# lightalchemist/nonlocal-image-edit

Measured on AMD Instinct MI355X. Metric: megapixels/sec end-to-end enhance (4K img, m=200, K=50); device-resident input and output (host->host per SURVEY 8d: host_to_host.value), higher is better.
Workload: dtype f64; 1 GPU; cfg4: 4096x4096 synthetic luminance, 20x10 samples (p=200), K=50, T=10, L=4 layers; device-resident: the luminance plane is in HBM when the timed region starts and the 4 layer planes are left in HBM (no PCIe inside `value`); parallelism=single GPU, formulation=phi_free_tables, storage=fp64 tables, histograms, reductions and MFMA; fp32 output planes

## Files before the change

nonlocal-image-edit_amd/csrc/sorted.hip:

```cpp
#include "sorted_rows.h"

#include <algorithm>
#include <cmath>
#include <cstdlib>

namespace nlek {

namespace {
constexpr int kSortThreads = 256;

__device__ __forceinline__ double recip0_d(double s, double eps) {
    double r = __builtin_amdgcn_rcp(s);
    r = fma(fma(-s, r, 1.0), r, r);
    r = fma(fma(-s, r, 1.0), r, r);
    return (fabs(s) >= eps) ? r : 0.0;
}

__device__ __forceinline__ int block_sum256(int v, int* red) {
#pragma unroll
    for (int off = 32; off > 0; off >>= 1) v += __shfl_xor(v, off);
    __syncthreads();
    if ((threadIdx.x & 63) == 0) red[threadIdx.x >> 6] = v;
    __syncthreads();
    return red[0] + red[1] + red[2] + red[3];
// ... 429 lines not shown
            }
            const int ns = (NC - s0 < SL) ? NC - s0 : SL;
            const int nlev = lev_nt * 16, xlo = lev_t0 * 16;
            const float inv_nlev = 1.0f / (float)nlev;
            for (int i = tid; i < ns * nlev; i += kT) {
                const int bb = (int)(((float)i + 0.5f) * inv_nlev);
                const int xx = xlo + (i - bb * nlev);
                const int f0 = sfc[xx], f1 = sfc[xx + 1];
                double sum = 0.0;
                for (int t = f0; t < f1; ++t) sum += sP[t * PS + bb];
                hrow[(size_t)(s0 + bb) * kLevels + xx] = sum;
            }
            __syncthreads();
        }
        __builtin_amdgcn_s_setprio(0);
        if (!has_next) break;
        lrow = nrow;
        nrow = nnrow;
        dsc = dsc_n;
        dsc_n = dsc_nn;
#pragma unroll
        for (int b = 0; b < kMaxBlocks; ++b) idx[b] = idx_n[b];
    }
}

int sorted_grid(int nrows, const SortedRows& sr) {
    int ncu = 256;
    int dev = 0;
    if (hipGetDevice(&dev) == hipSuccess) (void)hipDeviceGetAttribute(&ncu, hipDeviceAttributeMultiprocessorCount, dev);
    return std::max(1, std::min(nrows, sr.wgs_per_cu * ncu));
}

bool sorted_recurrence(GridSpec gs, double hx, double* kappa) {
    const double cs = gs.colStep, umax = std::max<double>(gs.colOff, gs.W - 1 - gs.colOff), nC = gs.nSelCols;
    const double span = umax + nC * cs;
    const double m_e = span * span / (hx * hx);
    const double m_rho = (2.0 * cs * umax + (2.0 * nC + 1.0) * cs * cs) / (hx * hx);
    *kappa = std::exp(-2.0 * cs * cs / (hx * hx));
    return gs.nSelCols > 12 && m_e < 500.0 && m_rho < 500.0;
}

bool sorted_moments_ok(GridSpec gs, double hx) {
    const double cs = gs.colStep, umax = std::max<double>(gs.colOff, gs.W - 1 - gs.colOff), nC = gs.nSelCols;
    const double span = umax + nC * cs;
    return span * span / (hx * hx) < 500.0;
}

hipError_t sorted_pass(hipStream_t s, int mode, GridSpec gs, int row0, int nrows_local, const SortedRows& sr, const double* d_g,
                       double eps, double* d_ybuf, double* d_h, const double* d_cvec, const float* d_xvec) {
    const int nC = gs.nSelCols, lev_t0 = sr.lev_t0, lev_nt = sr.lev_nt;
    if (!tables_apply(gs) || gs.W > sorted_max_width() || lev_t0 < 0 || lev_nt < 1 || lev_t0 + lev_nt > kLevels / 16)
        return hipErrorInvalidValue;
    if (nrows_local <= 0) return hipSuccess;
    const size_t shm = sorted_lds_bytes(gs.W, (nC < 11 ? nC : 11) | 1);
    const int grid = sorted_grid(nrows_local, sr);
#define NLE_SP1(NCV, CFV)                                                                                                 \
    {                                                                                                                     \
        if (shm > 48 * 1024) {                                                                                            \
            hipError_t ea = hipFuncSetAttribute(reinterpret_cast<const void*>(k_sorted_pass<NCV, CFV>),                   \
                                                hipFuncAttributeMaxDynamicSharedMemorySize, (int)shm);                    \
            if (ea != hipSuccess) return ea;                                                                              \
        }                                                                                                                 \
        hipLaunchKernelGGL((k_sorted_pass<NCV, CFV>), dim3((unsigned)grid), dim3(kT), shm, s, mode, sr.scol, sr.desc,      \
                           sr.first, gs, row0, nrows_local, sr.E, d_g, eps, d_ybuf, d_h, d_cvec, d_xvec, sr.kappa, lev_t0, \
                           lev_nt);                                                                                       \
    }
#define NLE_SP(NCV)                                                                                                       \
    case NCV:                                                                                                             \
        if constexpr ((NCV) > 1) {                                                                                        \
            if (sr.mom) {                                                                                                 \
                NLE_SP1(NCV, 2)                                                                                           \
                break;                                                                                                    \
            }                                                                                                             \
        }                                                                                                                 \
        if constexpr ((NCV) > 12) {                                                                                       \
            if (sr.rec) NLE_SP1(NCV, 1) else NLE_SP1(NCV, 0)                                                              \
        } else {                                                                                                          \
            if (sr.rec) return hipErrorInvalidValue;                                                                      \
            NLE_SP1(NCV, 0)                                                                                               \
        }                                                                                                                 \
        break;
    switch (nC) {
        NLE_SP(1) NLE_SP(2) NLE_SP(3) NLE_SP(4) NLE_SP(5) NLE_SP(6) NLE_SP(7) NLE_SP(8) NLE_SP(9) NLE_SP(10) NLE_SP(11)
        NLE_SP(12) NLE_SP(13) NLE_SP(14) NLE_SP(15) NLE_SP(16) NLE_SP(17) NLE_SP(18) NLE_SP(19) NLE_SP(20)
        NLE_SP(21) NLE_SP(22) NLE_SP(23) NLE_SP(24) NLE_SP(25) NLE_SP(26) NLE_SP(27) NLE_SP(28) NLE_SP(29)
        NLE_SP(30) NLE_SP(31) NLE_SP(32) NLE_SP(33) NLE_SP(34) NLE_SP(35) NLE_SP(36)
        default: return hipErrorInvalidValue;
    }
#undef NLE_SP
#undef NLE_SP1
    return hipGetLastError();
}

constexpr int kExpLayers = 4;
template <int NC, int kExpL, bool REC>
__global__ __launch_bounds__(kT) void k_sorted_expand(const unsigned short* __restrict__ scol, const uint2* __restrict__ desc,
                                                      GridSpec gs, int nrows, const double* __restrict__ Etab,
                                                      const double* __restrict__ g, size_t gstride, int nl,
                                                      const double* __restrict__ cvec, float* __restrict__ out,
                                                      long long ostride, double kappa, int round8) {
    extern __shared__ __attribute__((aligned(16))) unsigned char smem_raw[];
    constexpr int n = kLevels * NC;
    const int W = gs.W;
    double* sE = reinterpret_cast<double*>(smem_raw);
    float* sOut = reinterpret_cast<float*>(sE + ((W + 2) & ~1));
    const int tid = threadIdx.x;
    for (int i = tid; i <= W; i += kT) sE[i] = Etab[i];
    const int cb0 = gs.colOff, cs = gs.colStep;
    const unsigned sEa = lds_addr(sE);
    const size_t pitch = sorted_row_pitch(W);
    __syncthreads();
    for (int lrow = blockIdx.x; lrow < nrows; lrow += gridDim.x) {
        const uint2 dsc = desc[(size_t)lrow * kT + tid];
        const int len = dsc_len(dsc), x = dsc_level(dsc);
        const uint2* slot = reinterpret_cast<const uint2*>(scol + (size_t)lrow * pitch + (size_t)tid * dsc_chp(dsc));
        uint2 idx[kMaxBlocks];
#pragma unroll
        for (int b = 0; b < kMaxBlocks; ++b) {
            uint2 v = make_uint2(0u, 0u);
            if (4 * b < len) v = slot[b];
            idx[b] = v;
        }
        double gv[kExpL][NC];
#pragma unroll
        for (int l = 0; l < kExpL; ++l)
#pragma unroll
            for (int b = 0; b < NC; ++b) gv[l][b] = (l < nl) ? g[(size_t)l * gstride + (size_t)lrow * n + b * kLevels + x] : 0.0;
        const double* cv_row = cvec + (size_t)lrow * W;
        int wlen = len;
#pragma unroll
        for (int off = 32; off > 0; off >>= 1) wlen = max(wlen, __shfl_xor(wlen, off));
        wlen = __builtin_amdgcn_readfirstlane(wlen);
        auto pixel = [&](const unsigned c8, const bool on) {
            const unsigned c = c8 >> 3;
            const double cv = cv_row[c];
            double e[NC];
            column_factors<NC, REC>(sEa, c8, cb0, cs, kappa, [&](const int b, const double ev) { e[b] = ev; });
#pragma unroll
            for (int l = 0; l < kExpL; ++l) {
                double s0 = 0.0, s1 = 0.0;
#pragma unroll
                for (int b = 0; b < NC; ++b) {
                    if (b & 1) s1 += e[b] * gv[l][b];
                    else s0 += e[b] * gv[l][b];
                }
                if (on && l < nl) {
                    double v = cv * (s0 + s1);
                    if (round8) v = rint(fmin(255.0, fmax(0.0, v)));
                    sOut[l * W + c] = (float)v;
                }
            }
        };
#pragma unroll
        for (int b = 0; b < kMaxBlocks; ++b) {
            if (4 * b >= wlen) break;
            pixel(idx[b].x & 0xffffu, 4 * b < len);
            NLE_PIXEL_FENCE();
            if (4 * b + 1 < wlen) {
                pixel(idx[b].x >> 16, 4 * b + 1 < len);
                NLE_PIXEL_FENCE();
            }
            if (4 * b + 2 < wlen) {
                pixel(idx[b].y & 0xffffu, 4 * b + 2 < len);
                NLE_PIXEL_FENCE();
            }
            if (4 * b + 3 < wlen) {
                pixel(idx[b].y >> 16, 4 * b + 3 < len);
                NLE_PIXEL_FENCE();
            }
        }
        __syncthreads();
        for (int l = 0; l < nl; ++l) {
            float* orow = out + (size_t)l * ostride + (size_t)lrow * W;
            for (int c = tid; c < W; c += kT) orow[c] = sOut[l * W + c];
        }
        __syncthreads();
    }
}

int sorted_expand_layers(GridSpec gs) { return (gs.nSelCols <= 12 && gs.W <= 4096) ? kExpLayers : 2; }

hipError_t sorted_expand(hipStream_t s, GridSpec gs, int nrows_local, const SortedRows& sr, const double* d_g, size_t gstride,
                         int nl, const double* d_cvec, float* d_out, long long ostride, bool round8) {
    const int nC = gs.nSelCols;
    const int lmax = sorted_expand_layers(gs);
    if (!tables_apply(gs) || gs.W > sorted_max_width() || nl < 1 || nl > lmax) return hipErrorInvalidValue;
    if (nrows_local <= 0) return hipSuccess;
    const size_t shm = (size_t)((gs.W + 2) & ~1) * sizeof(double) + (size_t)lmax * gs.W * sizeof(float);
    int ncu = 256, dev = 0;
    if (hipGetDevice(&dev) == hipSuccess) (void)hipDeviceGetAttribute(&ncu, hipDeviceAttributeMultiprocessorCount, dev);
    const int grid = std::max(1, std::min(nrows_local, ncu));
#define NLE_SX1(NCV, LV, RECV)                                                                                         \
    {                                                                                                                  \
        if (shm > 48 * 1024) {                                                                                         \
            hipError_t ea = hipFuncSetAttribute(reinterpret_cast<const void*>(k_sorted_expand<NCV, LV, RECV>),         \
                                                hipFuncAttributeMaxDynamicSharedMemorySize, (int)shm);                 \
            if (ea != hipSuccess) return ea;                                                                           \
        }                                                                                                              \
        hipLaunchKernelGGL((k_sorted_expand<NCV, LV, RECV>), dim3((unsigned)grid), dim3(kT), shm, s, sr.scol, sr.desc, \
                           gs, nrows_local, sr.E, d_g, gstride, nl, d_cvec, d_out, ostride, sr.kappa, round8 ? 1 : 0); \
    }
#define NLE_SX(NCV)                                                                                                    \
    case NCV:                                                                                                          \
        if constexpr ((NCV) <= 12) {                                                                                   \
            if (lmax == kExpLayers) NLE_SX1(NCV, kExpLayers, false) else NLE_SX1(NCV, 2, false)                        \
        } else {                                                                                                       \
            if (sr.rec) NLE_SX1(NCV, 2, true) else NLE_SX1(NCV, 2, false)                                              \
        }                                                                                                              \
        break;
    switch (nC) {
        NLE_SX(1) NLE_SX(2) NLE_SX(3) NLE_SX(4) NLE_SX(5) NLE_SX(6) NLE_SX(7) NLE_SX(8) NLE_SX(9) NLE_SX(10) NLE_SX(11)
        NLE_SX(12) NLE_SX(13) NLE_SX(14) NLE_SX(15) NLE_SX(16) NLE_SX(17) NLE_SX(18) NLE_SX(19) NLE_SX(20) NLE_SX(21)
        NLE_SX(22) NLE_SX(23) NLE_SX(24) NLE_SX(25) NLE_SX(26) NLE_SX(27) NLE_SX(28) NLE_SX(29) NLE_SX(30) NLE_SX(31)
        NLE_SX(32) NLE_SX(33) NLE_SX(34) NLE_SX(35) NLE_SX(36)
        default: return hipErrorInvalidValue;
    }
#undef NLE_SX
#undef NLE_SX1
    return hipGetLastError();
}

template <int NC, bool REC>
__global__ __launch_bounds__(kT) void k_sorted_gram(const unsigned short* __restrict__ scol, const uint2* __restrict__ desc,
                                                    const unsigned short* __restrict__ first, GridSpec gs, int nrows,
                                                    const double* __restrict__ Etab, const double* __restrict__ cvec,
                                                    double* __restrict__ Aout, double kappa) {
    extern __shared__ __attribute__((aligned(16))) unsigned char smem_raw[];
    constexpr int NP = NC * (NC + 1) / 2;
    constexpr int SL = 11, PS = SL;
// ... 305 lines not shown
```

nonlocal-image-edit_amd/csrc/sorted_planes.hip:

```cpp
#include "sorted_rows.h"

#include <algorithm>

namespace nlek {

__host__ __device__ constexpr int planes_waves_per_simd(int nc, int np) { return nc * np <= 28 ? 4 : 2; }

template <int NC, int CF, int NP>
__global__ __launch_bounds__(kT, planes_waves_per_simd(NC, NP)) void k_sorted_reduce_planes(
    const unsigned short* __restrict__ scol, const uint2* __restrict__ desc, const unsigned short* __restrict__ first, GridSpec gs,
    int row0, int nrows, const double* __restrict__ Etab, const double* __restrict__ cvec, PlaneGroup pg, double kappa,
    int lev_t0, int lev_nt) {
#pragma clang fp contract(off)
    extern __shared__ __attribute__((aligned(16))) unsigned char smem_raw[];
    constexpr int n = kLevels * NC;
    constexpr int SL = NC < 11 ? NC : 11;
    constexpr int PS = SL | 1;
    constexpr bool REC = CF == 1, MOM = CF == 2;
    static_assert(!MOM || NC > 1, "the moment form needs two columns");
    const int W = gs.W;
    const size_t pitch = sorted_row_pitch(W);
    double* sE = reinterpret_cast<double*>(smem_raw);
    double* sP = sE + ((W + 2) & ~1);
    unsigned short* sfirst = reinterpret_cast<unsigned short*>(sP + (size_t)kT * PS);
    double* sCk = reinterpret_cast<double*>(sfirst + 2 * 260);
    const int tid = threadIdx.x;
    for (int i = tid; i <= W; i += kT) sE[i] = Etab[i];
    if (MOM && tid == 0) {
        double ck = 1.0, kp = 1.0;
        for (int b = 0; b < NC; ++b) {
            sCk[b] = ck;
            ck *= kp;
            kp *= kappa;
        }
    }
    const int cb0 = gs.colOff, cs = gs.colStep;
    const unsigned sEa = lds_addr(sE);

    const int G = (int)gridDim.x;
    int lrow = blockIdx.x, nrow = lrow + G;
    uint2 dsc = desc[(size_t)lrow * kT + tid];
    uint2 dsc_n = dsc;
    if (nrow < nrows) dsc_n = desc[(size_t)nrow * kT + tid];
    if (tid < 258) sfirst[tid] = first[(size_t)lrow * 258 + tid];
    uint2 idx[kMaxBlocks];
    auto load_idx = [&](uint2 (&dst)[kMaxBlocks], const int row, const uint2 d) {
        const uint2* slot = reinterpret_cast<const uint2*>(scol + (size_t)row * pitch + (size_t)tid * dsc_chp(d));
        const int ln = dsc_len(d);
#pragma unroll
        for (int b = 0; b < kMaxBlocks; ++b) {
            uint2 v = make_uint2(0u, 0u);
            if (4 * b < ln) v = slot[b];
            dst[b] = v;
        }
    };
    load_idx(idx, lrow, dsc);
    __syncthreads();
    for (int par = 0;; par ^= 1) {
        const bool has_next = nrow < nrows;
        const int nnrow = nrow + G;
        const unsigned short* sfc = sfirst + par * 260;
        const int len = dsc_len(dsc);
        double acc[NP][NC];
#pragma unroll
        for (int m = 0; m < NP; ++m)
#pragma unroll
            for (int b = 0; b < NC; ++b) acc[m][b] = 0.0;
        const double* cv_row = cvec + (size_t)lrow * W;
        const float* xv_row[NP];
#pragma unroll
        for (int m = 0; m < NP; ++m) xv_row[m] = pg.x[m] + (size_t)(row0 + lrow) * W;
        uint2 dsc_nn = dsc_n;
        unsigned short sf_n = 0;
        uint2 idx_n[kMaxBlocks];
        if (has_next) {
            if (nnrow < nrows) dsc_nn = desc[(size_t)nnrow * kT + tid];
            sf_n = first[(size_t)nrow * 258 + (tid < 258 ? tid : 257)];
            load_idx(idx_n, nrow, dsc_n);
        }
        auto pixel_mom = [&](const unsigned c8, const int at) {
            if constexpr (!MOM) return;
            else {
                const double e0 = e_at(sEa, c8, (unsigned)cb0 << 3);
                double rho = e_at(sEa, c8, (unsigned)(cb0 + cs) << 3);
                const bool keep = at < len;
                const double cv = cv_row[c8 >> 3];
                float xs[NP];
#pragma unroll
                for (int m = 0; m < NP; ++m) xs[m] = xv_row[m][c8 >> 3];
                double r0 = __builtin_amdgcn_rcp(e0);
                r0 = fma(fma(-e0, r0, 1.0), r0, r0);
                r0 = fma(fma(-e0, r0, 1.0), r0, r0);
                rho = rho * r0;
                const double rho2 = rho * rho;
#pragma unroll
                for (int m = 0; m < NP; ++m) {
                    double y = cv * (double)xs[m];
                    y = keep ? y : 0.0;
                    double te = y * e0;
                    acc[m][0] = fma(y, e0, acc[m][0]);
                    double to = te * rho;
                    acc[m][1] = fma(te, rho, acc[m][1]);
#pragma unroll
                    for (int b = 2; b < NC; b += 2) {
                        acc[m][b] = fma(te, rho2, acc[m][b]);
                        te = te * rho2;
                        if (b + 1 < NC) {
                            acc[m][b + 1] = fma(to, rho2, acc[m][b + 1]);
                            to = to * rho2;
                        }
                    }
                }
            }
        };
        auto pixel = [&](const unsigned c8, const bool on) {
            const double cv = cv_row[c8 >> 3];
            double y[NP];
#pragma unroll
            for (int m = 0; m < NP; ++m) {
                const double v = cv * (double)xv_row[m][c8 >> 3];
                y[m] = on ? v : 0.0;
            }
            column_factors<NC, REC>(sEa, c8, cb0, cs, kappa, [&](const int b, const double ev) {
#pragma unroll
                for (int m = 0; m < NP; ++m) acc[m][b] = fma(ev, y[m], acc[m][b]);
            });
        };
        int wlen = len;
#pragma unroll
        for (int off = 32; off > 0; off >>= 1) wlen = max(wlen, __shfl_xor(wlen, off));
        wlen = __builtin_amdgcn_readfirstlane(wlen);
#pragma unroll
        for (int b = 0; b < kMaxBlocks; ++b) {
            if (4 * b >= wlen) break;
            const unsigned cs4[4] = {idx[b].x & 0xffffu, idx[b].x >> 16, idx[b].y & 0xffffu, idx[b].y >> 16};
#pragma unroll
            for (int k = 0; k < 4; ++k) {
                if (4 * b + k < wlen) {
                    if constexpr (MOM) pixel_mom(cs4[k], 4 * b + k);
                    else pixel(cs4[k], 4 * b + k < len);
                    NLE_PIXEL_FENCE();
                }
            }
        }
        if constexpr (MOM) {
#pragma unroll
            for (int m = 0; m < NP; ++m)
#pragma unroll
                for (int b = 2; b < NC; ++b) acc[m][b] = acc[m][b] * sCk[b];
        }
        __builtin_amdgcn_s_setprio(3);
        const int nlev = lev_nt * 16, xlo = lev_t0 * 16;
        const float inv_nlev = 1.0f / (float)nlev;
#pragma unroll
        for (int m = 0; m < NP; ++m) {
            double* hrow = pg.h[m] + (size_t)lrow * n;
#pragma unroll
            for (int s0 = 0; s0 < NC; s0 += SL) {
#pragma unroll
                for (int i = 0; i < SL; ++i) sP[tid * PS + i] = (s0 + i < NC) ? acc[m][s0 + i] : 0.0;
                __syncthreads();
                if (m == 0 && s0 == 0) {
                    asm volatile("" ::"v"(sf_n), "v"(dsc_nn.x), "v"(dsc_nn.y));
#pragma unroll
                    for (int b = 0; b < kMaxBlocks; ++b) asm volatile("" ::"v"(idx_n[b].x), "v"(idx_n[b].y));
                    if (has_next && tid < 258) sfirst[(par ^ 1) * 260 + tid] = sf_n;
                }
                const int ns = (NC - s0 < SL) ? NC - s0 : SL;
                for (int i = tid; i < ns * nlev; i += kT) {
                    const int bb = (int)(((float)i + 0.5f) * inv_nlev);
                    const int xx = xlo + (i - bb * nlev);
                    const int f0 = sfc[xx], f1 = sfc[xx + 1];
                    double sum = 0.0;
                    for (int t = f0; t < f1; ++t) sum += sP[t * PS + bb];
                    hrow[(size_t)(s0 + bb) * kLevels + xx] = sum;
                }
                __syncthreads();
            }
        }
        __builtin_amdgcn_s_setprio(0);
        if (!has_next) break;
        lrow = nrow;
        nrow = nnrow;
        dsc = dsc_n;
        dsc_n = dsc_nn;
#pragma unroll
        for (int b = 0; b < kMaxBlocks; ++b) idx[b] = idx_n[b];
    }
}

int sorted_planes_per_launch(GridSpec gs) { return gs.nSelCols <= 12 ? kPlanesPerLaunch : 2; }

hipError_t sorted_reduce_planes(hipStream_t s, GridSpec gs, int row0, int nrows_local, const SortedRows& sr, const double* d_cvec,
                                const PlaneGroup& pg, int np) {
    const int nC = gs.nSelCols, lev_t0 = sr.lev_t0, lev_nt = sr.lev_nt;
    if (!tables_apply(gs) || gs.W > sorted_max_width() || lev_t0 < 0 || lev_nt < 1 || lev_t0 + lev_nt > kLevels / 16 || np < 2 ||
        np > sorted_planes_per_launch(gs))
        return hipErrorInvalidValue;
    if (nrows_local <= 0) return hipSuccess;
    const size_t shm = sorted_lds_bytes(gs.W, (nC < 11 ? nC : 11) | 1);
    SortedRows one = sr;
    if (planes_waves_per_simd(nC, np) < 4) one.wgs_per_cu = 1;
    const int grid = sorted_grid(nrows_local, one);
#define NLE_RP1(NCV, CFV, NPV)                                                                                            \
    {                                                                                                                     \
        if (shm > 48 * 1024) {                                                                                            \
            hipError_t ea = hipFuncSetAttribute(reinterpret_cast<const void*>(k_sorted_reduce_planes<NCV, CFV, NPV>),     \
                                                hipFuncAttributeMaxDynamicSharedMemorySize, (int)shm);                    \
            if (ea != hipSuccess) return ea;                                                                              \
        }                                                                                                                 \
        hipLaunchKernelGGL((k_sorted_reduce_planes<NCV, CFV, NPV>), dim3((unsigned)grid), dim3(kT), shm, s, sr.scol,       \
                           sr.desc, sr.first, gs, row0, nrows_local, sr.E, d_cvec, pg, sr.kappa, lev_t0, lev_nt);         \
    }
#define NLE_RPN(NCV, CFV)                                                                                                 \
    {                                                                                                                     \
        if constexpr ((NCV) <= 12) {                                                                                      \
            if (np == 4) NLE_RP1(NCV, CFV, 4) else if (np == 3) NLE_RP1(NCV, CFV, 3) else NLE_RP1(NCV, CFV, 2)            \
        } else {                                                                                                          \
            NLE_RP1(NCV, CFV, 2)                                                                                          \
        }                                                                                                                 \
    }
#define NLE_RP(NCV)                                                                                                       \
    case NCV:                                                                                                             \
        if constexpr ((NCV) > 1) {                                                                                        \
            if (sr.mom) {                                                                                                 \
                NLE_RPN(NCV, 2)                                                                                           \
                break;                                                                                                    \
            }                                                                                                             \
        }                                                                                                                 \
        if constexpr ((NCV) > 12) {                                                                                       \
            if (sr.rec) NLE_RPN(NCV, 1) else NLE_RPN(NCV, 0)                                                              \
        } else {                                                                                                          \
            if (sr.rec) return hipErrorInvalidValue;                                                                      \
            NLE_RPN(NCV, 0)                                                                                               \
        }                                                                                                                 \
        break;
    switch (nC) {
        NLE_RP(1) NLE_RP(2) NLE_RP(3) NLE_RP(4) NLE_RP(5) NLE_RP(6) NLE_RP(7) NLE_RP(8) NLE_RP(9) NLE_RP(10) NLE_RP(11)
        NLE_RP(12) NLE_RP(13) NLE_RP(14) NLE_RP(15) NLE_RP(16) NLE_RP(17) NLE_RP(18) NLE_RP(19) NLE_RP(20)
        NLE_RP(21) NLE_RP(22) NLE_RP(23) NLE_RP(24) NLE_RP(25) NLE_RP(26) NLE_RP(27) NLE_RP(28) NLE_RP(29)
        NLE_RP(30) NLE_RP(31) NLE_RP(32) NLE_RP(33) NLE_RP(34) NLE_RP(35) NLE_RP(36)
        default: return hipErrorInvalidValue;
    }
#undef NLE_RP
#undef NLE_RPN
#undef NLE_RP1
    return hipGetLastError();
}

}
```

nonlocal-image-edit_amd/csrc/tables.hip:

```cpp
#include "kernels.h"

#include <algorithm>

namespace nlek {

typedef double f64x4 __attribute__((ext_vector_type(4)));

constexpr int kLevels = 256;

constexpr int kGroupMin = 12;
constexpr int kGroupRounds = 3;

template <int CTRL, int ROW_MASK>
__device__ __forceinline__ double dpp_f64(double v) {
    int lo = __double2loint(v), hi = __double2hiint(v);
    lo = __builtin_amdgcn_update_dpp(0, lo, CTRL, ROW_MASK, 0xf, true);
    hi = __builtin_amdgcn_update_dpp(0, hi, CTRL, ROW_MASK, 0xf, true);
    return __hiloint2double(hi, lo);
}
__device__ __forceinline__ double wave_sum63(double v) {
    v += dpp_f64<0xB1, 0xf>(v);
    v += dpp_f64<0x4E, 0xf>(v);
    v += dpp_f64<0x141, 0xf>(v);
    v += dpp_f64<0x140, 0xf>(v);
// ... 51 lines not shown
    __shared__ int s_bad[4];
    if ((threadIdx.x & 63) == 0) {
        s_tiles[threadIdx.x >> 6] = tiles;
        s_bad[threadIdx.x >> 6] = any_bad ? 1 : 0;
    }
    __syncthreads();
    if (threadIdx.x == 0) {
        if (s_bad[0] | s_bad[1] | s_bad[2] | s_bad[3]) atomicOr(flag, 1);
        atomicOr(flag + 1, (int)(s_tiles[0] | s_tiles[1] | s_tiles[2] | s_tiles[3]));
    }
}

hipError_t check_levels(hipStream_t s, const float* d_lum, long long n, int* d_flag) {
    hipError_t e = hipMemsetAsync(d_flag, 0, 2 * sizeof(int), s);
    if (e != hipSuccess) return e;
    long long g = (n + 255) / 256;
    if (g > 1024) g = 1024;
    hipLaunchKernelGGL(k_check_levels, dim3((unsigned)g), dim3(256), 0, s, d_lum, n, d_flag);
    return hipGetLastError();
}

__global__ void k_hist_tables(GridSpec gs, const Sample4* __restrict__ samples, int p, double inv_hx2,
                              double inv_hy2, int row0, int nrows_local, double* __restrict__ er,
                              double* __restrict__ ecT, double* __restrict__ Ep) {
    const long long n_er = (long long)nrows_local * gs.nSelRows, n_ec = (long long)gs.nSelCols * gs.W,
                    n_ep = (long long)kLevels * p;
    for (long long i = (long long)blockIdx.x * blockDim.x + threadIdx.x; i < n_er + n_ec + n_ep;
         i += (long long)gridDim.x * blockDim.x) {
        if (i < n_er) {
            const int r = row0 + (int)(i / gs.nSelRows), a = (int)(i % gs.nSelRows);
            const double d = (double)(r - (gs.rowOff + a * gs.rowStep));
            er[i] = exp(-(d * d) * inv_hx2);
        } else if (i < n_er + n_ec) {
            const long long j = i - n_er;
            const int b = (int)(j / gs.W), c = (int)(j % gs.W);
            const double d = (double)(c - (gs.colOff + b * gs.colStep));
            ecT[j] = exp(-(d * d) * inv_hx2);
        } else {
            const long long j = i - n_er - n_ec;
            const int x = (int)(j / p), sidx = (int)(j % p);
            const double d = (double)x - (double)samples[sidx].z;
            Ep[j] = exp(-(d * d) * inv_hy2);
        }
    }
}

hipError_t hist_tables(hipStream_t s, GridSpec gs, const Sample4* d_samples, int p, double hx, double hy, int row0,
                       int nrows_local, double* d_er, double* d_ecT, double* d_Ep) {
    hipLaunchKernelGGL(k_hist_tables, dim3(256), dim3(256), 0, s, gs, d_samples, p, 1.0 / (hx * hx), 1.0 / (hy * hy),
                       row0, nrows_local, d_er, d_ecT, d_Ep);
    return hipGetLastError();
}

__global__ __launch_bounds__(256) void k_hist_g(GridSpec gs, int p, int nrows, int tiles_per_wave, int lev_t0, int lev_nt,
                                                const double* __restrict__ er, const double* __restrict__ Ep,
                                                const double* __restrict__ w, double* __restrict__ g) {
    extern __shared__ __attribute__((aligned(16))) unsigned char smem_raw[];
    double* sEr = reinterpret_cast<double*>(smem_raw);
    const int nC = gs.nSelCols, nR = gs.nSelRows, n = kLevels * nC;
    const int tid = threadIdx.x, lane = tid & 63, wave = tid >> 6, l15 = lane & 15, kq = lane >> 4;
    const int t0 = blockIdx.y * tiles_per_wave, ntiles = (nrows + 15) >> 4;
    const int rbase = t0 * 16, rcount = min(nrows - rbase, tiles_per_wave * 16);
    for (int i = tid; i < rcount * nR; i += 256) sEr[i] = er[(size_t)rbase * nR + i];
    const int q = blockIdx.x * 4 + wave;
    const bool col_ok = q < nC * lev_nt;
    const int b = col_ok ? q / lev_nt : 0, x = (lev_t0 + (col_ok ? q % lev_nt : 0)) * 16 + l15;
    const int col = b * kLevels + x;
    double bop[8];
#pragma unroll
    for (int ks = 0; ks < 8; ++ks) {
        const int a = ks * 4 + kq;
        bop[ks] = (col_ok && a < nR) ? w[a * nC + b] * Ep[(size_t)x * p + a * nC + b] : 0.0;
    }
    __syncthreads();
    if (!col_ok) return;
    const int ksteps = (nR + 3) >> 2;
    for (int t = t0; t < min(ntiles, t0 + tiles_per_wave); ++t) {
        const int rl = (t - t0) * 16 + l15;
        double aop[8];
#pragma unroll
        for (int ks = 0; ks < 8; ++ks) {
            const int a = ks * 4 + kq;
            aop[ks] = (ks < ksteps && rl < rcount && a < nR) ? sEr[rl * nR + a] : 0.0;
        }
        f64x4 acc = f64x4{0.0, 0.0, 0.0, 0.0};
#pragma unroll
        for (int ks = 0; ks < 8; ++ks)
            if (ks < ksteps) acc = __builtin_amdgcn_mfma_f64_16x16x4f64(aop[ks], bop[ks], acc, 0, 0, 0);
        if (col_ok) {
#pragma unroll
            for (int e = 0; e < 4; ++e) {
                const int ro = t * 16 + kq + 4 * e;
                if (ro < nrows) g[(size_t)ro * n + col] = acc[e];
            }
        }
    }
}

static hipError_t launch_hist_g(hipStream_t s, GridSpec gs, int p, int nrows_local, const double* d_er, const double* d_Ep,
                                const double* d_w, double* d_g, int lev_t0 = 0, int lev_nt = kLevels / 16) {
    const int ntiles = (nrows_local + 15) / 16;
    const int gx = (gs.nSelCols * lev_nt + 3) / 4;
    const int cap = gs.nSelRows > 24 ? 8 : 16;
    const int chunks = std::max(1, std::min(ntiles, std::max((640 + gx - 1) / gx, (ntiles + cap - 1) / cap)));
    const int tpw = (ntiles + chunks - 1) / chunks;
    const size_t shm = (size_t)tpw * 16 * gs.nSelRows * sizeof(double);
    if (shm > 48 * 1024) {
        hipError_t ea = hipFuncSetAttribute(reinterpret_cast<const void*>(k_hist_g), hipFuncAttributeMaxDynamicSharedMemorySize,
                                            (int)shm);
        if (ea != hipSuccess) return ea;
    }
    hipLaunchKernelGGL(k_hist_g, dim3((unsigned)gx, (unsigned)((ntiles + tpw - 1) / tpw)), dim3(256), shm, s, gs, p,
                       nrows_local, tpw, lev_t0, lev_nt, d_er, d_Ep, d_w, d_g);
    return hipGetLastError();
}

constexpr int kPixThreads = 512;
template <int NC>
__global__ __launch_bounds__(kPixThreads) void k_hist_pix(int mode, const float* __restrict__ lum, GridSpec gs, int row0,
                                                  const double* __restrict__ ecT, const double* __restrict__ g,
                                                  double eps, double* __restrict__ ybuf, double* __restrict__ hout,
                                                  const double* __restrict__ cvec, const float* __restrict__ xvec) {
    extern __shared__ __attribute__((aligned(16))) unsigned char smem_raw[];
    constexpr int n = kLevels * NC;
    constexpr int NS = NC | 1;
    const int W = gs.W;
    double* sg = reinterpret_cast<double*>(smem_raw);
    double* sh = sg + kLevels * NS;
    const int tid = threadIdx.x, lrow = blockIdx.x, r = row0 + lrow;
    const double* grow = g + (size_t)lrow * n;
    for (int i = tid; i < n; i += kPixThreads) {
        const int bb = i / kLevels, xx = i & (kLevels - 1);
        sh[xx * NS + bb] = 0.0;
        sg[xx * NS + bb] = (mode == ROWPASS_RECIP) ? grow[i] : 0.0;
    }
    __syncthreads();
    const int dr = r - gs.rowOff;
    const bool sample_row = dr >= 0 && (dr % gs.rowStep) == 0 && (dr / gs.rowStep) < gs.nSelRows;
    for (int c0 = 0; c0 < W; c0 += kPixThreads) {
        const bool inside = c0 + tid < W;
        const int c = inside ? c0 + tid : W - 1;
        const int x = (int)lum[(size_t)r * W + c];
        bool smp = !inside;
        if (sample_row) {
            const int dc = c - gs.colOff;
            smp = smp || (dc >= 0 && (dc % gs.colStep) == 0 && (dc / gs.colStep) < NC);
        }
        double e[NC];
#pragma unroll
        for (int b = 0; b < NC; ++b) e[b] = ecT[(size_t)b * W + c];
        double y = 1.0;
        if (mode == ROWPASS_XVEC) {
            y = cvec[(size_t)lrow * W + c] * (double)xvec[(size_t)r * W + c];
        } else if (mode == ROWPASS_RECIP) {
            double gv[NC];
#pragma unroll
            for (int b = 0; b < NC; ++b) gv[b] = sg[x * NS + b];
            double s0 = 0.0, s1 = 0.0;
#pragma unroll
            for (int b = 0; b < NC; ++b) {
                if (b & 1) s1 += e[b] * gv[b];
                else s0 += e[b] * gv[b];
            }
            y = recip_or_zero_d(s0 + s1, eps);
        }
        if (smp) y = 0.0;
// ... 275 lines not shown
        }
        switch (nC) {
            NLE_HP(1) NLE_HP(2) NLE_HP(3) NLE_HP(4) NLE_HP(5) NLE_HP(6) NLE_HP(7) NLE_HP(8) NLE_HP(9) NLE_HP(10) NLE_HP(11)
            NLE_HP(12) NLE_HP(13) NLE_HP(14) NLE_HP(15) NLE_HP(16) NLE_HP(17) NLE_HP(18) NLE_HP(19) NLE_HP(20)
            NLE_HP(21) NLE_HP(22) NLE_HP(23) NLE_HP(24) NLE_HP(25) NLE_HP(26) NLE_HP(27) NLE_HP(28) NLE_HP(29)
            NLE_HP(30) NLE_HP(31) NLE_HP(32) NLE_HP(33) NLE_HP(34) NLE_HP(35) NLE_HP(36)
            default: return hipErrorInvalidValue;
        }
#undef NLE_HP
    }
    Scope sc(obs, SUB_HIST_HH);
    return launch_hist_hh_z(s, v, d_h, d_HH, d_z);
}

size_t apply_reduce_planes_workspace_elems(GridSpec gs, int nrows_local, int np) {
    return hist_tiled_workspace_elems(gs, nrows_local) + (size_t)std::max(np - 2, 0) * nrows_local * kLevels * gs.nSelCols;
}

hipError_t apply_reduce_planes(hipStream_t s, const TableView& v, const float* const* d_x, int np, double* d_ws, double* d_m,
                               LaunchObserver* obs) {
    if (!tables_apply(v.gs) || v.sorted == nullptr || np < 2 || np > sorted_planes_per_launch(v.gs)) return hipErrorInvalidValue;
    const size_t tab = (size_t)v.nrows * kLevels * v.gs.nSelCols;
    double* d_HH = d_ws + (size_t)np * tab;
    PlaneGroup pg{};
    for (int m = 0; m < np; ++m) pg.x[m] = d_x[m], pg.h[m] = d_ws + (size_t)m * tab;
    if (obs) obs->begin(SUB_HIST_PIX);
    hipError_t ep = sorted_reduce_planes(s, v.gs, v.row0, v.nrows, *v.sorted, v.cvec, pg, np);
    if (obs) obs->end();
    if (ep != hipSuccess) return ep;
    for (int m = 0; m < np; ++m) {
        if (obs) obs->begin(SUB_HIST_HH);
        hipError_t eh = launch_hist_hh_z(s, v, pg.h[m], d_HH, d_m + (size_t)m * v.ldp);
        if (obs) obs->end();
        if (eh != hipSuccess) return eh;
    }
    return hipSuccess;
}

int apply_layers_per_launch(const TableView& v) {
    if (v.sorted != nullptr) return sorted_expand_layers(v.gs);
    const size_t table = (size_t)kLevels * (v.gs.nSelCols | 1) * sizeof(double);
    return (int)std::max<size_t>(1, std::min<size_t>(kDotLayers, (size_t)(144 * 1024) / table));
}

hipError_t apply_hist_layers(hipStream_t s, const TableView& v, const double* d_wl, int ldw, int nl, double* d_ws, float* d_out,
                             long long ostride, LaunchObserver* obs, bool round8) {
    if (v.nrows <= 0) return hipSuccess;
    if (!tables_apply(v.gs) || nl < 1 || nl > apply_layers_per_launch(v)) return hipErrorInvalidValue;
    const GridSpec gs = v.gs;
    const int nC = gs.nSelCols, p = v.p, row0 = v.row0, nrows_local = v.nrows;
    const SortedRows* sorted = v.sorted;
    const size_t n = (size_t)kLevels * nC, gstride = (size_t)nrows_local * n;
    if (obs) obs->begin(SUB_HIST_G);
    for (int l = 0; l < nl; ++l) {
        hipError_t eg = launch_hist_g(s, gs, p, nrows_local, v.er, v.Ep, d_wl + (size_t)l * ldw, d_ws + (size_t)l * gstride,
                                      sorted ? sorted->lev_t0 : 0, sorted ? sorted->lev_nt : kLevels / 16);
        if (eg != hipSuccess) return eg;
    }
    if (obs) obs->end(), obs->begin(SUB_HIST_PIX);
    if (sorted != nullptr) {
        hipError_t ex = sorted_expand(s, gs, nrows_local, *sorted, d_ws, gstride, nl, v.cvec, d_out, ostride, round8);
        if (obs) obs->end();
        return ex;
    }
#define NLE_HD(NCV)                                                                                                  \
    case NCV: {                                                                                                      \
        const size_t shm_d = (size_t)nl * kLevels * ((NCV) | 1) * sizeof(double);                                    \
        if (shm_d > 48 * 1024) {                                                                                     \
            hipError_t ea = hipFuncSetAttribute(reinterpret_cast<const void*>(k_hist_dot<NCV>),                      \
                                                hipFuncAttributeMaxDynamicSharedMemorySize, (int)shm_d);             \
            if (ea != hipSuccess) return ea;                                                                         \
        }                                                                                                            \
        hipLaunchKernelGGL((k_hist_dot<NCV>), dim3((unsigned)nrows_local), dim3(kDotThreads), shm_d, s, v.lum, gs,   \
                           row0, v.ecT, d_ws, gstride, nl, v.cvec, d_out, ostride, round8 ? 1 : 0);                  \
    } break;
    switch (nC) {
        NLE_HD(1) NLE_HD(2) NLE_HD(3) NLE_HD(4) NLE_HD(5) NLE_HD(6) NLE_HD(7) NLE_HD(8) NLE_HD(9) NLE_HD(10) NLE_HD(11)
        NLE_HD(12) NLE_HD(13) NLE_HD(14) NLE_HD(15) NLE_HD(16) NLE_HD(17) NLE_HD(18) NLE_HD(19) NLE_HD(20)
        NLE_HD(21) NLE_HD(22) NLE_HD(23) NLE_HD(24) NLE_HD(25) NLE_HD(26) NLE_HD(27) NLE_HD(28) NLE_HD(29)
        NLE_HD(30) NLE_HD(31) NLE_HD(32) NLE_HD(33) NLE_HD(34) NLE_HD(35) NLE_HD(36)
        default: return hipErrorInvalidValue;
    }
#undef NLE_HD
    if (obs) obs->end();
    return hipGetLastError();
}

hipError_t apply_small(hipStream_t s, int p, int K, int ldk, int L, int ldw, const double* d_m, const double* d_D,
                       const double* d_Vrows, const double* d_xA, const double* d_resp, double* d_t, double* d_Wp,
                       double* d_YA) {
    const size_t shm = (size_t)(2 * p + K + 256) * sizeof(double);
    hipLaunchKernelGGL(k_apply_small, dim3((unsigned)L), dim3(256), shm, s, p, K, ldk, L, ldw, d_m, d_D, d_Vrows, d_xA,
                       d_resp, d_t, d_Wp, d_YA);
    return hipGetLastError();
}

hipError_t scatter_samples(hipStream_t s, int p, int L, const long long* d_loc, const double* d_YA, float* d_Y,
                           long long ystride, bool round8) {
    hipLaunchKernelGGL(k_scatter_samples, dim3((unsigned)((L * p + 255) / 256)), dim3(256), 0, s, p, L, d_loc, d_YA, d_Y,
                       ystride, round8 ? 1 : 0);
    return hipGetLastError();
}

__device__ __forceinline__ int tri_index(int i, int j, int n) {
    return i * n - (i * (i - 1)) / 2 + (j - i);
}

constexpr int kGhistRowsThreads = 512;
__global__ __launch_bounds__(kGhistRowsThreads) void k_ghist_rows(const float* __restrict__ lum, GridSpec gs, int row0,
// ... 362 lines not shown
```

Before: 3460 MP/s.

## Prefetch cvec/x gathers ahead in sorted kernels and batch hist_g across layers

The sorted expand kernel now software-pipelines the next row's descriptor, index, g-table and cvec gathers so they load while the current row's pixels are computed. The single-plane XVEC row pass is routed through the planes reducer, which gains an NP=1 path that gathers cvec and x one block ahead. k_hist_g is templated on layer count so up to 4 layers share one launch and one Ep load. These changes aim to hide gather latency and cut launches, at the cost of more registers and possible occupancy loss.

After: 3471 MP/s, median of 2. No clear change (+0.3%).

```diff
diff --git a/nonlocal-image-edit_amd/csrc/sorted.hip b/nonlocal-image-edit_amd/csrc/sorted.hip
--- a/nonlocal-image-edit_amd/csrc/sorted.hip
+++ b/nonlocal-image-edit_amd/csrc/sorted.hip
@@ -505,6 +505,12 @@
     if (!tables_apply(gs) || gs.W > sorted_max_width() || lev_t0 < 0 || lev_nt < 1 || lev_t0 + lev_nt > kLevels / 16)
         return hipErrorInvalidValue;
     if (nrows_local <= 0) return hipSuccess;
+    if (mode == ROWPASS_XVEC) {
+        if (d_cvec == nullptr || d_xvec == nullptr || d_ybuf != nullptr) return hipErrorInvalidValue;
+        PlaneGroup pg{};
+        pg.x[0] = d_xvec, pg.h[0] = d_h;
+        return sorted_reduce_planes(s, gs, row0, nrows_local, sr, d_cvec, pg, 1);
+    }
     const size_t shm = sorted_lds_bytes(gs.W, (nC < 11 ? nC : 11) | 1);
     const int grid = sorted_grid(nrows_local, sr);
 #define NLE_SP1(NCV, CFV)                                                                                                 \
@@ -554,6 +560,10 @@
                                                       long long ostride, double kappa, int round8) {
     extern __shared__ __attribute__((aligned(16))) unsigned char smem_raw[];
     constexpr int n = kLevels * NC;
+    constexpr int NB = kExpL == kExpLayers ? 4 : kMaxBlocks;
+    constexpr bool PIPE = NC <= 29 || (NC == 30 && REC);
+    constexpr bool CVALL = NC <= 12;
+    constexpr int NCR = CVALL ? 4 * NB : 4;
     const int W = gs.W;
     double* sE = reinterpret_cast<double*>(smem_raw);
     float* sOut = reinterpret_cast<float*>(sE + ((W + 2) & ~1));
@@ -562,31 +572,87 @@
     const int cb0 = gs.colOff, cs = gs.colStep;
     const unsigned sEa = lds_addr(sE);
     const size_t pitch = sorted_row_pitch(W);
-    __syncthreads();
-    for (int lrow = blockIdx.x; lrow < nrows; lrow += gridDim.x) {
-        const uint2 dsc = desc[(size_t)lrow * kT + tid];
-        const int len = dsc_len(dsc), x = dsc_level(dsc);
-        const uint2* slot = reinterpret_cast<const uint2*>(scol + (size_t)lrow * pitch + (size_t)tid * dsc_chp(dsc));
-        uint2 idx[kMaxBlocks];
-#pragma unroll
-        for (int b = 0; b < kMaxBlocks; ++b) {
+    auto load_idx = [&](uint2 (&dst)[NB], const int row, const uint2 d) {
+        const uint2* slot = reinterpret_cast<const uint2*>(scol + (size_t)row * pitch + (size_t)tid * dsc_chp(d));
+        const int ln = dsc_len(d);
+#pragma unroll
+        for (int b = 0; b < NB; ++b) {
             uint2 v = make_uint2(0u, 0u);
-            if (4 * b < len) v = slot[b];
-            idx[b] = v;
-        }
-        double gv[kExpL][NC];
-#pragma unroll
-        for (int l = 0; l < kExpL; ++l)
-#pragma unroll
-            for (int b = 0; b < NC; ++b) gv[l][b] = (l < nl) ? g[(size_t)l * gstride + (size_t)lrow * n + b * kLevels + x] : 0.0;
+            if (4 * b < ln) v = slot[b];
+            dst[b] = v;
+        }
+    };
+    auto load_gv = [&](double (&dst)[kExpL][NC], const int row, const uint2 d) {
+        const double* gx = g + (size_t)row * n + dsc_level(d);
+#pragma unroll
+        for (int l = 0; l < kExpL; ++l) {
+            const double* gl = gx + (l < nl ? (size_t)l * gstride : (size_t)0);
+#pragma unroll
+            for (int b = 0; b < NC; ++b) dst[l][b] = gl[b * kLevels];
+        }
+    };
+    auto gather4 = [&](double* dst, const double* cv_row, const uint2 ix) {
+        dst[0] = cv_row[(ix.x & 0xffffu) >> 3];
+        dst[1] = cv_row[ix.x >> 19];
+        dst[2] = cv_row[(ix.y & 0xffffu) >> 3];
+        dst[3] = cv_row[ix.y >> 19];
+    };
+    auto gather_first = [&](double (&dst)[NCR], const int row, const uint2 (&ix)[NB], const int wl) {
+        const double* cv_row = cvec + (size_t)row * W;
+#pragma unroll
+        for (int b = 0; b < (CVALL ? NB : 1); ++b) {
+            if (4 * b >= wl) break;
+            gather4(&dst[4 * b], cv_row, ix[b]);
+        }
+    };
+    auto wave_len = [&](const uint2 d) {
+        int wl = dsc_len(d);
+#pragma unroll
+        for (int off = 32; off > 0; off >>= 1) wl = max(wl, __shfl_xor(wl, off));
+        return __builtin_amdgcn_readfirstlane(wl);
+    };
+    const int G = (int)gridDim.x;
+    int lrow = blockIdx.x, nrow = lrow + G;
+    uint2 dsc = desc[(size_t)lrow * kT + tid];
+    uint2 dsc_n = dsc;
+    if constexpr (PIPE) {
+        if (nrow < nrows) dsc_n = desc[(size_t)nrow * kT + tid];
+    }
+    uint2 idx[NB];
+    load_idx(idx, lrow, dsc);
+    int wlen = wave_len(dsc);
+    double cvr[NCR];
+    if constexpr (PIPE) gather_first(cvr, lrow, idx, wlen);
+    double gv[kExpL][NC];
+    load_gv(gv, lrow, dsc);
+    __syncthreads();
+    for (;;) {
+        const bool has_next = nrow < nrows;
+        const int nnrow = nrow + G;
+        const int len = dsc_len(dsc);
+        uint2 dsc_nn = dsc_n;
+        uint2 idx_n[PIPE ? NB : 1];
+        if constexpr (PIPE) {
+#pragma unroll
+            for (int l = 0; l < kExpL; ++l)
+#pragma unroll
+                for (int b = 0; b < NC; ++b) asm volatile("" ::"v"(gv[l][b]));
+#pragma unroll
+            for (int i = 0; i < NCR; ++i) {
+                if (4 * (i / 4) < wlen) asm volatile("" ::"v"(cvr[i]));
+            }
+            if (has_next) {
+                if (nnrow < nrows) dsc_nn = desc[(size_t)nnrow * kT + tid];
+                load_idx(idx_n, nrow, dsc_n);
+            } else {
+#pragma unroll
+                for (int b = 0; b < NB; ++b) idx_n[b] = make_uint2(0u, 0u);
+            }
+        }
         const double* cv_row = cvec + (size_t)lrow * W;
-        int wlen = len;
-#pragma unroll
-        for (int off = 32; off > 0; off >>= 1) wlen = max(wlen, __shfl_xor(wlen, off));
-        wlen = __builtin_amdgcn_readfirstlane(wlen);
-        auto pixel = [&](const unsigned c8, const bool on) {
+        auto pixel = [&](const unsigned c8, const bool on, const double cv_reg) {
             const unsigned c = c8 >> 3;
-            const double cv = cv_row[c];
+            const double cv = PIPE ? cv_reg : cv_row[c];
             double e[NC];
             column_factors<NC, REC>(sEa, c8, cb0, cs, kappa, [&](const int b, const double ev) { e[b] = ev; });
 #pragma unroll
@@ -605,21 +671,44 @@
             }
         };
 #pragma unroll
-        for (int b = 0; b < kMaxBlocks; ++b) {
+        for (int b = 0; b < NB; ++b) {
             if (4 * b >= wlen) break;
-            pixel(idx[b].x & 0xffffu, 4 * b < len);
+            double cvb[4];
+            if constexpr (PIPE && !CVALL) {
+                if (b + 1 < NB && 4 * (b + 1) < wlen) gather4(cvb, cv_row, idx[b + 1]);
+            }
+            double cv4[4] = {0.0, 0.0, 0.0, 0.0};
+            if constexpr (PIPE) {
+#pragma unroll
+                for (int k = 0; k < 4; ++k) cv4[k] = cvr[(CVALL ? 4 * b : 0) + k];
+            }
+            pixel(idx[b].x & 0xffffu, 4 * b < len, cv4[0]);
             NLE_PIXEL_FENCE();
             if (4 * b + 1 < wlen) {
-                pixel(idx[b].x >> 16, 4 * b + 1 < len);
+                pixel(idx[b].x >> 16, 4 * b + 1 < len, cv4[1]);
                 NLE_PIXEL_FENCE();
             }
             if (4 * b + 2 < wlen) {
-                pixel(idx[b].y & 0xffffu, 4 * b + 2 < len);
+                pixel(idx[b].y & 0xffffu, 4 * b + 2 < len, cv4[2]);
                 NLE_PIXEL_FENCE();
             }
             if (4 * b + 3 < wlen) {
-                pixel(idx[b].y >> 16, 4 * b + 3 < len);
+                pixel(idx[b].y >> 16, 4 * b + 3 < len, cv4[3]);
                 NLE_PIXEL_FENCE();
+            }
+            if constexpr (PIPE && !CVALL) {
+                if (b + 1 < NB && 4 * (b + 1) < wlen) {
+#pragma unroll
+                    for (int k = 0; k < 4; ++k) cvr[k] = cvb[k];
+                }
+            }
+        }
+        int wlen_n = 0;
+        if constexpr (PIPE) {
+            if (has_next) {
+                wlen_n = wave_len(dsc_n);
+                gather_first(cvr, nrow, idx_n, wlen_n);
+                load_gv(gv, nrow, dsc_n);
             }
         }
         __syncthreads();
@@ -628,6 +717,21 @@
             for (int c = tid; c < W; c += kT) orow[c] = sOut[l * W + c];
         }
         __syncthreads();
+        if (!has_next) break;
+        lrow = nrow;
+        nrow = nnrow;
+        if constexpr (PIPE) {
+            dsc = dsc_n;
+            dsc_n = dsc_nn;
+            wlen = wlen_n;
+#pragma unroll
+            for (int b = 0; b < NB; ++b) idx[b] = idx_n[b];
+        } else {
+            dsc = desc[(size_t)lrow * kT + tid];
+            load_idx(idx, lrow, dsc);
+            load_gv(gv, lrow, dsc);
+            wlen = wave_len(dsc);
+        }
     }
 }
 
diff --git a/nonlocal-image-edit_amd/csrc/sorted_planes.hip b/nonlocal-image-edit_amd/csrc/sorted_planes.hip
--- a/nonlocal-image-edit_amd/csrc/sorted_planes.hip
+++ b/nonlocal-image-edit_amd/csrc/sorted_planes.hip
@@ -4,7 +4,7 @@
 
 namespace nlek {
 
-__host__ __device__ constexpr int planes_waves_per_simd(int nc, int np) { return nc * np <= 28 ? 4 : 2; }
+__host__ __device__ constexpr int planes_waves_per_simd(int nc, int np) { return np == 1 ? (nc <= 12 ? 4 : 2) : (nc * np <= 28 ? 4 : 2); }
 
 template <int NC, int CF, int NP>
 __global__ __launch_bounds__(kT, planes_waves_per_simd(NC, NP)) void k_sorted_reduce_planes(
@@ -55,6 +55,31 @@
         }
     };
     load_idx(idx, lrow, dsc);
+    constexpr bool AHEAD = NP == 1;
+    auto gather4 = [&](double (&cv)[4], float (&xs)[NP][4], const int row, const uint2 ix) {
+        const unsigned c4[4] = {(ix.x & 0xffffu) >> 3, ix.x >> 19, (ix.y & 0xffffu) >> 3, ix.y >> 19};
+        const double* cv_row = cvec + (size_t)row * W;
+#pragma unroll
+        for (int k = 0; k < 4; ++k) cv[k] = cv_row[c4[k]];
+#pragma unroll
+        for (int m = 0; m < NP; ++m) {
+            const float* xv_row = pg.x[m] + (size_t)(row0 + row) * W;
+#pragma unroll
+            for (int k = 0; k < 4; ++k) xs[m][k] = xv_row[c4[k]];
+        }
+    };
+    auto wave_len = [&](const uint2 d) {
+        int wl = dsc_len(d);
+#pragma unroll
+        for (int off = 32; off > 0; off >>= 1) wl = max(wl, __shfl_xor(wl, off));
+        return __builtin_amdgcn_readfirstlane(wl);
+    };
+    int wlen = wave_len(dsc);
+    double cvc[4] = {};
+    float xsc[NP][4] = {};
+    if constexpr (AHEAD) {
+        if (wlen > 0) gather4(cvc, xsc, lrow, idx[0]);
+    }
     __syncthreads();
     for (int par = 0;; par ^= 1) {
         const bool has_next = nrow < nrows;
@@ -70,6 +95,14 @@
         const float* xv_row[NP];
 #pragma unroll
         for (int m = 0; m < NP; ++m) xv_row[m] = pg.x[m] + (size_t)(row0 + lrow) * W;
+        if (AHEAD && wlen > 0) {
+#pragma unroll
+            for (int k = 0; k < 4; ++k) {
+                asm volatile("" ::"v"(cvc[k]));
+#pragma unroll
+                for (int m = 0; m < NP; ++m) asm volatile("" ::"v"(xsc[m][k]));
+            }
+        }
         uint2 dsc_nn = dsc_n;
         unsigned short sf_n = 0;
         uint2 idx_n[kMaxBlocks];
@@ -78,16 +111,21 @@
             sf_n = first[(size_t)nrow * 258 + (tid < 258 ? tid : 257)];
             load_idx(idx_n, nrow, dsc_n);
         }
-        auto pixel_mom = [&](const unsigned c8, const int at) {
+        auto pixel_mom = [&](const unsigned c8, const int at, const double cva, const float (&xsa)[NP]) {
             if constexpr (!MOM) return;
             else {
                 const double e0 = e_at(sEa, c8, (unsigned)cb0 << 3);
                 double rho = e_at(sEa, c8, (unsigned)(cb0 + cs) << 3);
                 const bool keep = at < len;
-                const double cv = cv_row[c8 >> 3];
+                double cv = cva;
                 float xs[NP];
 #pragma unroll
-                for (int m = 0; m < NP; ++m) xs[m] = xv_row[m][c8 >> 3];
+                for (int m = 0; m < NP; ++m) xs[m] = xsa[m];
+                if constexpr (!AHEAD) {
+                    cv = cv_row[c8 >> 3];
+#pragma unroll
+                    for (int m = 0; m < NP; ++m) xs[m] = xv_row[m][c8 >> 3];
+                }
                 double r0 = __builtin_amdgcn_rcp(e0);
                 r0 = fma(fma(-e0, r0, 1.0), r0, r0);
                 r0 = fma(fma(-e0, r0, 1.0), r0, r0);
@@ -113,12 +151,15 @@
                 }
             }
         };
-        auto pixel = [&](const unsigned c8, const bool on) {
-            const double cv = cv_row[c8 >> 3];
+        auto pixel = [&](const unsigned c8, const bool on, const double cva, const float (&xsa)[NP]) {
+            double cv = cva;
+            if constexpr (!AHEAD) cv = cv_row[c8 >> 3];
             double y[NP];
 #pragma unroll
             for (int m = 0; m < NP; ++m) {
-                const double v = cv * (double)xv_row[m][c8 >> 3];
+                float x = xsa[m];
+                if constexpr (!AHEAD) x = xv_row[m][c8 >> 3];
+                const double v = cv * (double)x;
                 y[m] = on ? v : 0.0;
             }
             column_factors<NC, REC>(sEa, c8, cb0, cs, kappa, [&](const int b, const double ev) {
@@ -126,20 +167,31 @@
                 for (int m = 0; m < NP; ++m) acc[m][b] = fma(ev, y[m], acc[m][b]);
             });
         };
-        int wlen = len;
-#pragma unroll
-        for (int off = 32; off > 0; off >>= 1) wlen = max(wlen, __shfl_xor(wlen, off));
-        wlen = __builtin_amdgcn_readfirstlane(wlen);
 #pragma unroll
         for (int b = 0; b < kMaxBlocks; ++b) {
             if (4 * b >= wlen) break;
+            const bool more = AHEAD && b + 1 < kMaxBlocks && 4 * (b + 1) < wlen;
+            double cvn[4];
+            float xsn[NP][4];
+            if (more) gather4(cvn, xsn, lrow, idx[b + 1]);
             const unsigned cs4[4] = {idx[b].x & 0xffffu, idx[b].x >> 16, idx[b].y & 0xffffu, idx[b].y >> 16};
 #pragma unroll
             for (int k = 0; k < 4; ++k) {
                 if (4 * b + k < wlen) {
-                    if constexpr (MOM) pixel_mom(cs4[k], 4 * b + k);
-                    else pixel(cs4[k], 4 * b + k < len);
+                    float xs[NP];
+#pragma unroll
+                    for (int m = 0; m < NP; ++m) xs[m] = xsc[m][k];
+                    if constexpr (MOM) pixel_mom(cs4[k], 4 * b + k, cvc[k], xs);
+                    else pixel(cs4[k], 4 * b + k < len, cvc[k], xs);
                     NLE_PIXEL_FENCE();
+                }
+            }
+            if (more) {
+#pragma unroll
+                for (int k = 0; k < 4; ++k) {
+                    cvc[k] = cvn[k];
+#pragma unroll
+                    for (int m = 0; m < NP; ++m) xsc[m][k] = xsn[m][k];
                 }
             }
         }
@@ -152,6 +204,7 @@
         __builtin_amdgcn_s_setprio(3);
         const int nlev = lev_nt * 16, xlo = lev_t0 * 16;
         const float inv_nlev = 1.0f / (float)nlev;
+        const int wlen_n = wave_len(dsc_n);
 #pragma unroll
         for (int m = 0; m < NP; ++m) {
             double* hrow = pg.h[m] + (size_t)lrow * n;
@@ -165,6 +218,7 @@
 #pragma unroll
                     for (int b = 0; b < kMaxBlocks; ++b) asm volatile("" ::"v"(idx_n[b].x), "v"(idx_n[b].y));
                     if (has_next && tid < 258) sfirst[(par ^ 1) * 260 + tid] = sf_n;
+                    if (AHEAD && has_next && wlen_n > 0) gather4(cvc, xsc, nrow, idx_n[0]);
                 }
                 const int ns = (NC - s0 < SL) ? NC - s0 : SL;
                 for (int i = tid; i < ns * nlev; i += kT) {
@@ -184,6 +238,7 @@
         nrow = nnrow;
         dsc = dsc_n;
         dsc_n = dsc_nn;
+        wlen = wlen_n;
 #pragma unroll
         for (int b = 0; b < kMaxBlocks; ++b) idx[b] = idx_n[b];
     }
@@ -194,7 +249,7 @@
 hipError_t sorted_reduce_planes(hipStream_t s, GridSpec gs, int row0, int nrows_local, const SortedRows& sr, const double* d_cvec,
                                 const PlaneGroup& pg, int np) {
     const int nC = gs.nSelCols, lev_t0 = sr.lev_t0, lev_nt = sr.lev_nt;
-    if (!tables_apply(gs) || gs.W > sorted_max_width() || lev_t0 < 0 || lev_nt < 1 || lev_t0 + lev_nt > kLevels / 16 || np < 2 ||
+    if (!tables_apply(gs) || gs.W > sorted_max_width() || lev_t0 < 0 || lev_nt < 1 || lev_t0 + lev_nt > kLevels / 16 || np < 1 ||
         np > sorted_planes_per_launch(gs))
         return hipErrorInvalidValue;
     if (nrows_local <= 0) return hipSuccess;
@@ -214,7 +269,7 @@
     }
 #define NLE_RPN(NCV, CFV)                                                                                                 \
     {                                                                                                                     \
-        if constexpr ((NCV) <= 12) {                                                                                      \
+        if (np == 1) NLE_RP1(NCV, CFV, 1) else if constexpr ((NCV) <= 12) {                                               \
             if (np == 4) NLE_RP1(NCV, CFV, 4) else if (np == 3) NLE_RP1(NCV, CFV, 3) else NLE_RP1(NCV, CFV, 2)            \
         } else {                                                                                                          \
             NLE_RP1(NCV, CFV, 2)                                                                                          \
diff --git a/nonlocal-image-edit_amd/csrc/tables.hip b/nonlocal-image-edit_amd/csrc/tables.hip
--- a/nonlocal-image-edit_amd/csrc/tables.hip
+++ b/nonlocal-image-edit_amd/csrc/tables.hip
@@ -127,9 +127,11 @@
     return hipGetLastError();
 }
 
+template <int NL>
 __global__ __launch_bounds__(256) void k_hist_g(GridSpec gs, int p, int nrows, int tiles_per_wave, int lev_t0, int lev_nt,
                                                 const double* __restrict__ er, const double* __restrict__ Ep,
-                                                const double* __restrict__ w, double* __restrict__ g) {
+                                                const double* __restrict__ w, int ldw, double* __restrict__ g,
+                                                size_t gstride) {
     extern __shared__ __attribute__((aligned(16))) unsigned char smem_raw[];
     double* sEr = reinterpret_cast<double*>(smem_raw);
     const int nC = gs.nSelCols, nR = gs.nSelRows, n = kLevels * nC;
@@ -141,11 +143,14 @@
     const bool col_ok = q < nC * lev_nt;
     const int b = col_ok ? q / lev_nt : 0, x = (lev_t0 + (col_ok ? q % lev_nt : 0)) * 16 + l15;
     const int col = b * kLevels + x;
-    double bop[8];
+    double bop[NL][8];
 #pragma unroll
     for (int ks = 0; ks < 8; ++ks) {
         const int a = ks * 4 + kq;
-        bop[ks] = (col_ok && a < nR) ? w[a * nC + b] * Ep[(size_t)x * p + a * nC + b] : 0.0;
+        const bool in = col_ok && a < nR;
+        const double ep = in ? Ep[(size_t)x * p + a * nC + b] : 0.0;
+#pragma unroll
+        for (int l = 0; l < NL; ++l) bop[l][ks] = in ? w[(size_t)l * ldw + a * nC + b] * ep : 0.0;
     }
     __syncthreads();
     if (!col_ok) return;
@@ -158,35 +163,46 @@
             const int a = ks * 4 + kq;
             aop[ks] = (ks < ksteps && rl < rcount && a < nR) ? sEr[rl * nR + a] : 0.0;
         }
-        f64x4 acc = f64x4{0.0, 0.0, 0.0, 0.0};
-#pragma unroll
-        for (int ks = 0; ks < 8; ++ks)
-            if (ks < ksteps) acc = __builtin_amdgcn_mfma_f64_16x16x4f64(aop[ks], bop[ks], acc, 0, 0, 0);
-        if (col_ok) {
+#pragma unroll
+        for (int l = 0; l < NL; ++l) {
+            f64x4 acc = f64x4{0.0, 0.0, 0.0, 0.0};
+#pragma unroll
+            for (int ks = 0; ks < 8; ++ks)
+                if (ks < ksteps) acc = __builtin_amdgcn_mfma_f64_16x16x4f64(aop[ks], bop[l][ks], acc, 0, 0, 0);
 #pragma unroll
             for (int e = 0; e < 4; ++e) {
                 const int ro = t * 16 + kq + 4 * e;
-                if (ro < nrows) g[(size_t)ro * n + col] = acc[e];
-            }
-        }
-    }
-}
-
+                if (ro < nrows) g[(size_t)l * gstride + (size_t)ro * n + col] = acc[e];
+            }
+        }
+    }
+}
+
+constexpr int kHistGLayers = 4;
 static hipError_t launch_hist_g(hipStream_t s, GridSpec gs, int p, int nrows_local, const double* d_er, const double* d_Ep,
-                                const double* d_w, double* d_g, int lev_t0 = 0, int lev_nt = kLevels / 16) {
+                                const double* d_w, double* d_g, int lev_t0 = 0, int lev_nt = kLevels / 16, int nl = 1,
+                                int ldw = 0, size_t gstride = 0) {
     const int ntiles = (nrows_local + 15) / 16;
     const int gx = (gs.nSelCols * lev_nt + 3) / 4;
     const int cap = gs.nSelRows > 24 ? 8 : 16;
     const int chunks = std::max(1, std::min(ntiles, std::max((640 + gx - 1) / gx, (ntiles + cap - 1) / cap)));
     const int tpw = (ntiles + chunks - 1) / chunks;
     const size_t shm = (size_t)tpw * 16 * gs.nSelRows * sizeof(double);
-    if (shm > 48 * 1024) {
-        hipError_t ea = hipFuncSetAttribute(reinterpret_cast<const void*>(k_hist_g), hipFuncAttributeMaxDynamicSharedMemorySize,
-                                            (int)shm);
-        if (ea != hipSuccess) return ea;
-    }
-    hipLaunchKernelGGL(k_hist_g, dim3((unsigned)gx, (unsigned)((ntiles + tpw - 1) / tpw)), dim3(256), shm, s, gs, p,
-                       nrows_local, tpw, lev_t0, lev_nt, d_er, d_Ep, d_w, d_g);
+#define NLE_HG(NLV)                                                                                                      \
+    case NLV: {                                                                                                          \
+        if (shm > 48 * 1024) {                                                                                           \
+            hipError_t ea = hipFuncSetAttribute(reinterpret_cast<const void*>(k_hist_g<NLV>),                            \
+                                                hipFuncAttributeMaxDynamicSharedMemorySize, (int)shm);                   \
+            if (ea != hipSuccess) return ea;                                                                             \
+        }                                                                                                                \
+        hipLaunchKernelGGL((k_hist_g<NLV>), dim3((unsigned)gx, (unsigned)((ntiles + tpw - 1) / tpw)), dim3(256), shm, s, \
+                           gs, p, nrows_local, tpw, lev_t0, lev_nt, d_er, d_Ep, d_w, ldw, d_g, gstride);                 \
+    } break;
+    switch (nl) {
+        NLE_HG(1) NLE_HG(2) NLE_HG(3) NLE_HG(4)
+        default: return hipErrorInvalidValue;
+    }
+#undef NLE_HG
     return hipGetLastError();
 }
 
@@ -568,9 +584,10 @@
     const SortedRows* sorted = v.sorted;
     const size_t n = (size_t)kLevels * nC, gstride = (size_t)nrows_local * n;
     if (obs) obs->begin(SUB_HIST_G);
-    for (int l = 0; l < nl; ++l) {
+    for (int l = 0; l < nl; l += kHistGLayers) {
         hipError_t eg = launch_hist_g(s, gs, p, nrows_local, v.er, v.Ep, d_wl + (size_t)l * ldw, d_ws + (size_t)l * gstride,
-                                      sorted ? sorted->lev_t0 : 0, sorted ? sorted->lev_nt : kLevels / 16);
+                                      sorted ? sorted->lev_t0 : 0, sorted ? sorted->lev_nt : kLevels / 16,
+                                      std::min(kHistGLayers, nl - l), ldw, gstride);
         if (eg != hipSuccess) return eg;
     }
     if (obs) obs->end(), obs->begin(SUB_HIST_PIX);
```
